# XiYe20/VPTR

Hardware: AMD Instinct MI355X
Metric: predicted frames/sec (train step) NAR KTH 10->10 @64x64 (higher is better)
Workload: dtype bf16x3 (split-bf16 MFMA, fp32 accumulate/storage); 1 GPU; K64: KTH 64x64x1 10->10, VPTREnc/Dec(528, Tanh, reflect) + VPTRFormerNAR(4 enc + 8 dec, d=528, 8 heads, ws 4, dropout 0.10), single_iter of train_NAR.py, random-init weights; per_gpu_batch=16, global_batch=16, frames_per_clip=10, parallelism=dp1, launch=hipGraph, dec_weight_grads=True, frozen_encoder_convs=winograd F(4x4,3x3), 36 strided-batch P16 products per convolution

## Files before the change

vptr_amd/_lib.py:

```python
import ctypes
import os

import torch

_HERE = os.path.dirname(os.path.abspath(__file__))
LIB_PATH = os.environ.get("VPTR_HIP_LIB") or os.path.join(_HERE, "libvptr_hip.so")

c_void_p, c_int, c_float, c_int64, c_uint32 = ctypes.c_void_p, ctypes.c_int, ctypes.c_float, ctypes.c_int64, ctypes.c_uint32


class GemmDesc(ctypes.Structure):
    _fields_ = [
        ("A", c_void_p), ("B", c_void_p), ("D", c_void_p), ("Dpre", c_void_p),
        ("lda", c_int64), ("ldb", c_int64), ("ldd", c_int64),
        ("M", c_int), ("N", c_int), ("K", c_int),
        ("a_mode", c_int), ("b_mode", c_int),
        ("precision", c_int), ("split_k", c_int), ("atomic", c_int),
        ("colscale", c_void_p), ("bias", c_void_p),
        ("alpha", c_float), ("act", c_int),
        ("rowscale", c_void_p), ("rs_div", c_int), ("rs_mod", c_int),
        ("dropout_p", c_float), ("seed_dev", c_void_p), ("site", c_uint32),
        ("residual", c_void_p), ("ldr", c_int64),
        ("act_after", c_int),
        ("conv_IH", c_int), ("conv_IW", c_int), ("conv_Cin", c_int), ("conv_OH", c_int), ("conv_OW", c_int),
        ("conv_KH", c_int), ("conv_KW", c_int), ("conv_stride", c_int), ("conv_pad", c_int), ("conv_pad_mode", c_int),
        ("conv_transposed", c_int),
        ("a_rowsum", c_void_p),
        ("batch", c_int), ("ksegs", c_int),
        ("A_x1", c_void_p), ("A_x2", c_void_p), ("B_x1", c_void_p), ("B_x2", c_void_p), ("D_x1", c_void_p), ("D_x2", c_void_p),
        ("bias_x1", c_void_p), ("bias_x2", c_void_p), ("alpha_x1", c_float), ("alpha_x2", c_float),
        ("D_planes", c_void_p),
        ("d_p16", c_int),
        ("act_grad_src", c_void_p),
        ("frame_stats", c_void_p), ("frame_rows", c_int),
        ("d_transposed", c_int),
        ("d_row_w", c_int), ("d_row_off", c_int),
        ("batch_accum", c_int),
        ("batch_stride_a", c_int64), ("batch_stride_b", c_int64), ("batch_stride_d", c_int64),
    ]


class ReduceEntry(ctypes.Structure):
    _fields_ = [("part", c_void_p), ("dst0", c_void_p), ("dst1", c_void_p), ("nparts", c_int), ("C", c_int)]


class WPlaneEntry(ctypes.Structure):
    _fields_ = [("W", c_void_p), ("Wp", c_void_p), ("WT", c_void_p), ("ldw", c_int64), ("N", c_int), ("K", c_int)]


P, I, F, L, U = c_void_p, c_int, c_float, c_int64, c_uint32
SIGNATURES = {
    "vptr_gemm": [ctypes.POINTER(GemmDesc), P],
    "vptr_gemm_tile_cols": [I],
    "vptr_split_planes": [P, P, L, I, P],
    "vptr_wino_in": [P, P, I, I, I, I, L, I, P],
    "vptr_wino_out": [P, P, P, P, P, I, I, I, I, L, I, I, P],
    "vptr_wino_out_in": [P, P, P, P, P, P, I, I, I, I, L, I, I, I, P],
    "vptr_to_p16": [P, P, L, I, P],
    "vptr_weight_planes": [P, P, I, I, P],
    "vptr_gemm_grouped": [ctypes.POINTER(GemmDesc), P, P, I, I, P],
    "vptr_layernorm_fwd": [P, P, P, P, P, P, I, I, P, P, I, I, F, I, P],
    "vptr_layernorm_bwd": [P, P, P, P, P, P, P, P, P, I, I, P, P],
    "vptr_layernorm_bwd_deferred": [P, P, P, P, P, P, P, I, I, P, P, P],
    "vptr_layernorm_bwd_partials": [I, I],
    "vptr_partial_reduce": [P, I, I, I, P],
    "vptr_rowmod_sum": [P, P, I, I, I, I, P],
    "vptr_colsum": [P, P, I, I, P],
    "vptr_window_copy": [P, P, I, I, I, I, I, I, I, I, P],
    "vptr_add_rowtab": [P, P, P, I, I, I, I, P],
    "vptr_winattn_fwd": [P, P, P, P, P, P, I, I, I, I, I, I, F, P, U, I, P],
    "vptr_winattn_bwd": [P, P, P, P, P, P, P, P, P, P, I, I, I, I, I, I, F, P, U, F, I, P],
    "vptr_winattn_bwd_ws": [P, P, P, P, P, P, P, P, P, P, I, I, I, I, I, I, F, P, U, F, I, P, I, P],
    "vptr_winattn_bwd_workspace": [I],
    "vptr_tattn_fwd": [P, P, P, P, I, I, I, I, I, I, I, F, P, U, I, P],
    "vptr_tattn_bwd": [P, P, P, P, P, P, P, I, I, I, I, I, I, I, F, P, U, F, I, P],
    "vptr_attn_route": [I, I, I, I, I, I, I, L, I, I, P, I],
    "vptr_tattn_step": [P, P, P, P, I, I, I, I, I, I, P],
    "vptr_tsattn_fwd": [P, P, P, P, I, I, I, I, I, I, I, I, F, P, U, I, P],
    "vptr_tsattn_bwd": [P, P, P, P, P, P, P, I, I, I, I, I, I, I, I, F, P, U, I, P],
    "vptr_colstats": [P, P, P, P, F, P, I, I, P],
    "vptr_colstats_running": [P, P, P, P, F, P, I, I, P, P, F, P, P],
    "vptr_groupstats": [P, P, P, P, F, I, I, P],
    "vptr_norm_act_fwd": [P, P, P, P, P, P, I, I, I, I, I, F, P, U, P, I, I, P, I, P, F, P],
    "vptr_norm_act_bwd": [P, P, P, P, P, P, P, P, P, P, I, I, I, I, I, I, F, P, U, P, I, I, I, P],
    "vptr_norm_act_bwd_deferred": [P, P, P, P, P, P, P, P, I, I, I, I, I, F, P, U, P, I, I, I, P, P],
    "vptr_norm_act_bwd_partials": [I, I, I, I],
    "vptr_dwconv3x3_fwd": [P, P, P, P, I, I, I, I, P, P],
    "vptr_dwconv3x3_bwd": [P, P, P, P, P, P, I, I, I, I, P],
    "vptr_dwconv3x3_norm_fwd": [P, P, P, P, F, I, P, P, P, P, P, P, I, I, I, I, P, P],
    "vptr_dwconv3x3_bwd_xh": [P, P, P, P, P, P, I, I, I, I, P],
    "vptr_nchw_to_tokens": [P, P, I, I, I, P],
    "vptr_tokens_to_nchw": [P, P, I, I, I, I, P],
    "vptr_nchw_to_tokens_masked": [P, P, P, I, I, I, P],
    "vptr_act_bwd": [P, P, P, I, I, I, F, P, I, I, F, P, U, I, P],
    "vptr_dropout": [P, P, L, F, P, U, P],
    "vptr_rowscale": [P, P, P, I, I, I, I, P],
    "vptr_conv7_in_fwd": [P, P, P, P, P, I, I, I, I, I, P],
    "vptr_conv7_in_fwd_planes": [P, P, P, P, P, I, I, I, I, I, P],
    "vptr_conv7_out_fwd": [P, P, P, P, I, I, I, I, I, I, P],
    "vptr_conv7_out_bwd_data": [P, P, P, P, I, I, I, I, I, I, P],
    "vptr_conv7_out_bwd_weight": [P, P, P, P, P, I, I, I, I, I, I, P],
    "vptr_conv7_out_bwd_weight_ws": [P, P, P, P, P, I, I, I, I, I, I, P, I, P],
    "vptr_conv7_out_bwd_weight_workspace": [I, I],
    "vptr_bnrelu_bwd": [P, P, P, P, L, I, P],
    "vptr_bnrelu_bwd_params": [P, P, P, P, P, P, L, I, P],
    "vptr_bnrelu_bwd_fused": [P, P, P, P, P, P, P, P, L, I, P],
    "vptr_im2col_nhwc": [P, P, I, I, I, I, I, I, I, I, I, I, I, P],
    "vptr_im2col_nhwc_p16": [P, P, I, I, I, I, I, I, I, I, I, I, I, P],
    "vptr_reflect_fold": [P, P, I, I, I, I, I, P],
    "vptr_conv7_in_bwd_weight": [P, P, P, I, I, I, I, I, P],
    "vptr_mse_gdl_fwd": [P, P, P, P, P, I, I, I, P],
    "vptr_mse_gdl_bwd": [P, P, P, P, P, I, I, I, P],
    "vptr_nce_fwd": [P, P, P, P, I, I, I, F, P],
    "vptr_nce_bwd": [P, P, P, P, P, P, I, I, I, F, P],
    "vptr_frame_metrics": [P, P, P, P, P, P, I, I, I, I, I, F, P],
    "vptr_frame_metrics_accumulate": [P, P, I, I, P],
    "vptr_clip_ingest": [P, P, P, P, P, P, P, P, P, I, I, I, I, I, I, I, I, I, I, I, I, I, I, P],
    "vptr_clip_panels": [P, P, P, P, P, P, P, P, I, I, I, I, I, I, I, I, I, P],
    "vptr_droppath_scales": [P, P, I, I, P, U, P],
    "vptr_sumsq": [P, L, P, P],
    "vptr_sumsq_ws": [P, L, P, P, I, P],
    "vptr_set_deterministic": [I],
    "vptr_get_deterministic": [],
    "vptr_wgrad_sync_stats": [P, P],
    "vptr_wgrad_kernel_counts": [P, I],
    "vptr_adamw": [P, P, P, P, L, F, F, F, F, F, P, P, F, F, P],
}
EXPORTS = sorted(list(SIGNATURES) + ["vptr_abi_version", "vptr_last_error"])
EXT_SIGNATURES = {
    "vptr_meters_add": [P, I, P, F, P],
}
OPTIM_SIGNATURES = {
    "vptr_optim_prepare": [P, P, P, P, P],
    "vptr_adamw_ctl": [P, P, P, P, L, P, P],
}
CONVFFN_SIGNATURES = {
    "vptr_norm_act_bwd_sums": [P, P, P, P, P, P, P, P, P, I, I, I, I, F, P, U, P, P],
    "vptr_dwconv3x3_norm_bwd": [P, P, P, P, P, P, P, I, F, P, U, P, P, P, P, P, I, I, I, I, I, P],
}


def _load():
    if not os.path.exists(LIB_PATH):
        raise ImportError(
            "vptr_amd: %s is missing. Build it with `python -m vptr_amd.build` (needs hipcc, gfx950). "
            "There is no CPU / PyTorch fallback for the VPTR hot path." % LIB_PATH)
    lib = ctypes.CDLL(LIB_PATH)
    for name, argt in list(SIGNATURES.items()) + list(EXT_SIGNATURES.items()) + list(OPTIM_SIGNATURES.items()) + list(CONVFFN_SIGNATURES.items()):
        fn = getattr(lib, name)
        fn.argtypes = argt
        fn.restype = c_int
    lib.vptr_abi_version.restype = c_int
    lib.vptr_last_error.restype = ctypes.c_char_p
    if lib.vptr_abi_version() != 10:
        raise ImportError("vptr_amd: ABI version mismatch in %s" % LIB_PATH)
    return lib


lib = _load()


def check(rc, what):
    if rc != 0:
        raise RuntimeError("%s failed (%d): %s" % (what, rc, lib.vptr_last_error().decode()))


def ptr(t):
    if t is None:
        return None
    return c_void_p(t.data_ptr())


def stream():
    return c_void_p(torch._C._cuda_getCurrentRawStream(torch.cuda.current_device()))


def require_cuda(*tensors):
    for t in tensors:
        if t is not None and not t.is_cuda:
            raise RuntimeError("vptr_amd ops run on the MI355X only (got a %s tensor); there is no CPU fallback" % t.device)
```

vptr_amd/build.py:

```python
import hashlib
import os
import subprocess
import sys
from concurrent.futures import ThreadPoolExecutor

HERE = os.path.dirname(os.path.abspath(__file__))
CSRC = os.path.join(HERE, "csrc")
OBJ = os.path.join(CSRC, "_build")
LIB = os.path.join(HERE, "libvptr_hip.so")
SOURCES = ["api.hip", "gemm.hip", "gemm_p16.hip", "layernorm.hip", "norm_act.hip", "dwconv.hip", "attn.hip", "attn_mfma.hip", "attn16.hip", "elementwise.hip", "conv7.hip", "losses.hip", "metrics.hip", "meters.hip", "optim.hip", "ingest.hip", "panels.hip", "winograd.hip"]
FLAGS = ["--offload-arch=gfx950", "-O3", "-std=c++17", "-fPIC", "-munsafe-fp-atomics", "-ffp-contract=fast", "-fno-slp-vectorize",
         "-Wno-unused-result"]


def _hipcc():
    for c in (os.environ.get("HIPCC"), "/opt/rocm/bin/hipcc", "hipcc"):
        if c and (os.path.isabs(c) and os.path.exists(c) or not os.path.isabs(c)):
            return c
    raise RuntimeError("hipcc not found")


def _digest(paths):
    h = hashlib.sha256()
    for p in paths:
        with open(p, "rb") as f:
            h.update(f.read())
    h.update(" ".join(FLAGS).encode())
    return h.hexdigest()


def _compile(src, force):
    obj = os.path.join(OBJ, src.replace(".hip", ".o"))
    stamp = obj + ".sha"
    deps = [os.path.join(CSRC, src), os.path.join(CSRC, "common.h"), os.path.join(CSRC, "gemm_shared.h"), os.path.join(CSRC, "attn_mfma.h"),
            os.path.join(CSRC, "attn_route.h"), os.path.join(HERE, "..", "include", "vptr_hip.h"), os.path.join(HERE, "..", "include", "vptr_hip_ext.h"),
            os.path.join(HERE, "..", "include", "vptr_hip_optim.h"), os.path.join(HERE, "..", "include", "vptr_hip_convffn.h")]
    dig = _digest(deps)
    if not force and os.path.exists(obj) and os.path.exists(stamp) and open(stamp).read() == dig:
        return obj, False
    cmd = [_hipcc()] + FLAGS + ["-c", os.path.join(CSRC, src), "-o", obj]
    r = subprocess.run(cmd, capture_output=True, text=True)
    if r.returncode != 0:
        raise RuntimeError("hipcc failed for %s:\n%s\n%s" % (src, r.stdout[-4000:], r.stderr[-8000:]))
    with open(stamp, "w") as f:
        f.write(dig)
    return obj, True


def build(force=False, verbose=True):
    os.makedirs(OBJ, exist_ok=True)
    with ThreadPoolExecutor(max_workers=min(8, len(SOURCES))) as ex:
        res = list(ex.map(lambda s: _compile(s, force), SOURCES))
    objs = [o for o, _ in res]
    if any(c for _, c in res) or not os.path.exists(LIB):
        cmd = [_hipcc(), "--offload-arch=gfx950", "-shared", "-fPIC", "-o", LIB] + objs
        r = subprocess.run(cmd, capture_output=True, text=True)
        if r.returncode != 0:
            raise RuntimeError("link failed:\n%s\n%s" % (r.stdout[-4000:], r.stderr[-8000:]))
        if verbose:
            print("built", LIB)
    elif verbose:
        print("up to date:", LIB)
    return LIB


if __name__ == "__main__":
    build(force="--force" in sys.argv)
```

vptr_amd/csrc/dwconv.hip:

```cpp
#include "common.h"
#include "../../include/vptr_hip_convffn.h"
#include <type_traits>

struct DwRow { float4 l, m, r; };
__device__ __forceinline__ float4 scale4(const float4 v, const float s) { return make_float4(v.x * s, v.y * s, v.z * s, v.w * s); }
__device__ __forceinline__ DwRow dw_load_row(const float4* __restrict__ x, int64_t frame_row0, int row, int H, int xw, int W, int F4,
                                             int c4) {
  const float rok = (row >= 0 && row < H) ? 1.f : 0.f;
  const int64_t base = (frame_row0 + min(max(row, 0), H - 1)) * W;
  DwRow o;
  o.l = scale4(x[(base + max(xw - 1, 0)) * F4 + c4], xw > 0 ? rok : 0.f);
  o.m = scale4(x[(base + xw) * F4 + c4], rok);
  o.r = scale4(x[(base + min(xw + 1, W - 1)) * F4 + c4], xw + 1 < W ? rok : 0.f);
  return o;
}
__device__ __forceinline__ void fma4(float4& a, const float4 w, const float4 v) {
  a.x += w.x * v.x; a.y += w.y * v.y; a.z += w.z * v.z; a.w += w.w * v.w;
}
__global__ __launch_bounds__(256) void dwconv_fwd_kernel(const float* __restrict__ x_, const float* __restrict__ w9,
                                                         const float* __restrict__ b, float* __restrict__ y_, int frames, int H,
                                                         int W, int F4, int flip) {
  const int64_t idx = (int64_t)blockIdx.x * 256 + threadIdx.x;
  if (idx >= (int64_t)frames * W * F4) return;
  const int c4 = (int)(idx % F4);
  const int xw = (int)((idx / F4) % W);
  const int64_t f = idx / ((int64_t)F4 * W);
  const float4* __restrict__ x = reinterpret_cast<const float4*>(x_);
  float4* __restrict__ y = reinterpret_cast<float4*>(y_);
  float4 w[9];
#pragma unroll
  for (int t = 0; t < 9; ++t) w[t] = reinterpret_cast<const float4*>(w9)[(int64_t)(flip ? 8 - t : t) * F4 + c4];
  const float4 bias = b ? reinterpret_cast<const float4*>(b)[c4] : make_float4(0.f, 0.f, 0.f, 0.f);
  DwRow r0 = dw_load_row(x, f * H, -1, H, xw, W, F4, c4), r1 = dw_load_row(x, f * H, 0, H, xw, W, F4, c4);
  for (int yh = 0; yh < H; ++yh) {
    const DwRow r2 = dw_load_row(x, f * H, yh + 1, H, xw, W, F4, c4);
    float4 a = bias;
    fma4(a, w[0], r0.l); fma4(a, w[1], r0.m); fma4(a, w[2], r0.r);
    fma4(a, w[3], r1.l); fma4(a, w[4], r1.m); fma4(a, w[5], r1.r);
    fma4(a, w[6], r2.l); fma4(a, w[7], r2.m); fma4(a, w[8], r2.r);
    y[((f * H + yh) * W + xw) * F4 + c4] = a;
    r0 = r1;
    r1 = r2;
  }
}

struct DwRow2 { float4 c0, c1, c2, c3; };
typedef __attribute__((ext_vector_type(4))) _Float16 half4_t;
__device__ __forceinline__ float4 dw_ld4(const float4* __restrict__ x, const int64_t i) { return x[i]; }
__device__ __forceinline__ float4 dw_ld4(const half4_t* __restrict__ x, const int64_t i) {
  const half4_t h = x[i];
  return make_float4((float)h.x, (float)h.y, (float)h.z, (float)h.w);
}
template <typename XT>
__device__ __forceinline__ DwRow2 dw_load_row2(const XT* __restrict__ x, int64_t frame_row0, int row, int H, int xw0, int W, int F4,
                                               int c4) {
  const float rok = (row >= 0 && row < H) ? 1.f : 0.f;
  const int64_t base = (frame_row0 + min(max(row, 0), H - 1)) * W;
  DwRow2 o;
  o.c0 = scale4(dw_ld4(x, (base + max(xw0 - 1, 0)) * F4 + c4), xw0 > 0 ? rok : 0.f);
  o.c1 = scale4(dw_ld4(x, (base + xw0) * F4 + c4), rok);
  o.c2 = scale4(dw_ld4(x, (base + xw0 + 1) * F4 + c4), rok);
  o.c3 = scale4(dw_ld4(x, (base + min(xw0 + 2, W - 1)) * F4 + c4), xw0 + 2 < W ? rok : 0.f);
  return o;
}
__global__ __launch_bounds__(256) void dwconv_fwd2_kernel(const float* __restrict__ x_, const float* __restrict__ w9,
                                                          const float* __restrict__ b, float* __restrict__ y_, int frames, int H,
                                                          int W, int F4, int flip, float* __restrict__ stats) {
  const int64_t idx = (int64_t)blockIdx.x * 256 + threadIdx.x;
  const int W2 = W >> 1;
  if (idx >= (int64_t)frames * W2 * F4) return;
  const int c4 = (int)(idx % F4);
  const int xw0 = (int)((idx / F4) % W2) * 2;
  const int64_t f = idx / ((int64_t)F4 * W2);
  const float4* __restrict__ x = reinterpret_cast<const float4*>(x_);
  float4* __restrict__ y = reinterpret_cast<float4*>(y_);
  float4 w[9];
#pragma unroll
  for (int t = 0; t < 9; ++t) w[t] = reinterpret_cast<const float4*>(w9)[(int64_t)(flip ? 8 - t : t) * F4 + c4];
  const float4 bias = b ? reinterpret_cast<const float4*>(b)[c4] : make_float4(0.f, 0.f, 0.f, 0.f);
  DwRow2 r0 = dw_load_row2(x, f * H, -1, H, xw0, W, F4, c4), r1 = dw_load_row2(x, f * H, 0, H, xw0, W, F4, c4);
  float ssum = 0.f, ssq = 0.f;
  for (int yh = 0; yh < H; ++yh) {
    const DwRow2 r2 = dw_load_row2(x, f * H, yh + 1, H, xw0, W, F4, c4);
    float4 a = bias, a2 = bias;
    fma4(a, w[0], r0.c0); fma4(a, w[1], r0.c1); fma4(a, w[2], r0.c2);
    fma4(a, w[3], r1.c0); fma4(a, w[4], r1.c1); fma4(a, w[5], r1.c2);
    fma4(a, w[6], r2.c0); fma4(a, w[7], r2.c1); fma4(a, w[8], r2.c2);
    fma4(a2, w[0], r0.c1); fma4(a2, w[1], r0.c2); fma4(a2, w[2], r0.c3);
    fma4(a2, w[3], r1.c1); fma4(a2, w[4], r1.c2); fma4(a2, w[5], r1.c3);
    fma4(a2, w[6], r2.c1); fma4(a2, w[7], r2.c2); fma4(a2, w[8], r2.c3);
    y[((f * H + yh) * W + xw0) * F4 + c4] = a;
    y[((f * H + yh) * W + xw0 + 1) * F4 + c4] = a2;
    if (stats) {
      ssum += ((a.x + a.y) + (a.z + a.w)) + ((a2.x + a2.y) + (a2.z + a2.w));
      ssq += ((a.x * a.x + a.y * a.y) + (a.z * a.z + a.w * a.w)) + ((a2.x * a2.x + a2.y * a2.y) + (a2.z * a2.z + a2.w * a2.w));
    }
    r0 = r1;
    r1 = r2;
  }
  if (stats) {
    const float S = wave_sum(ssum), Q = wave_sum(ssq);
    if ((threadIdx.x & 63) == 0) {
      unsafeAtomicAdd(stats + VPTR_FRAME_STATS_STRIDE * f, S);
      unsafeAtomicAdd(stats + VPTR_FRAME_STATS_STRIDE * f + 1, Q);
    }
  }
}
__device__ __forceinline__ float dpp_from_prev(float v) {
  return __int_as_float(__builtin_amdgcn_update_dpp(0, __float_as_int(v), 0x111, 0xf, 0xf, true));
}
__device__ __forceinline__ float dpp_from_next(float v) {
  return __int_as_float(__builtin_amdgcn_update_dpp(0, __float_as_int(v), 0x101, 0xf, 0xf, true));
}
__device__ __forceinline__ DwRow2 dw_load_row3(const float4* __restrict__ x, int64_t frame_row0, int row, int H, int xw0, int W, int F4,
                                               int c4, float lok, float rok_) {
  const float rok = (row >= 0 && row < H) ? 1.f : 0.f;
  const int64_t base = (frame_row0 + min(max(row, 0), H - 1)) * W;
  DwRow2 o;
  o.c1 = scale4(x[(base + xw0) * F4 + c4], rok);
  o.c2 = scale4(x[(base + xw0 + 1) * F4 + c4], rok);
  o.c0 = make_float4(dpp_from_prev(o.c2.x) * lok, dpp_from_prev(o.c2.y) * lok, dpp_from_prev(o.c2.z) * lok, dpp_from_prev(o.c2.w) * lok);
  o.c3 = make_float4(dpp_from_next(o.c1.x) * rok_, dpp_from_next(o.c1.y) * rok_, dpp_from_next(o.c1.z) * rok_, dpp_from_next(o.c1.w) * rok_);
  return o;
}
__global__ __launch_bounds__(256) void dwconv_fwd3_kernel(const float* __restrict__ x_, const float* __restrict__ w9,
                                                          const float* __restrict__ b, float* __restrict__ y_, int frames, int H,
                                                          int W, int F4, int flip, float* __restrict__ stats) {
  const int64_t idx = (int64_t)blockIdx.x * 256 + threadIdx.x;
  const int W2 = W >> 1;
  if (idx >= (int64_t)frames * W2 * F4) return;
  const int xp = (int)(idx % W2), xw0 = xp * 2;
  const int c4 = (int)((idx / W2) % F4);
  const int64_t f = idx / ((int64_t)F4 * W2);
  const float lok = xp > 0 ? 1.f : 0.f, rok_ = xp + 1 < W2 ? 1.f : 0.f;
  const float4* __restrict__ x = reinterpret_cast<const float4*>(x_);
  float4* __restrict__ y = reinterpret_cast<float4*>(y_);
  float4 w[9];
#pragma unroll
  for (int t = 0; t < 9; ++t) w[t] = reinterpret_cast<const float4*>(w9)[(int64_t)(flip ? 8 - t : t) * F4 + c4];
  const float4 bias = b ? reinterpret_cast<const float4*>(b)[c4] : make_float4(0.f, 0.f, 0.f, 0.f);
  DwRow2 r0 = dw_load_row3(x, f * H, -1, H, xw0, W, F4, c4, lok, rok_), r1 = dw_load_row3(x, f * H, 0, H, xw0, W, F4, c4, lok, rok_);
  float ssum = 0.f, ssq = 0.f;
  for (int yh = 0; yh < H; ++yh) {
    const DwRow2 r2 = dw_load_row3(x, f * H, yh + 1, H, xw0, W, F4, c4, lok, rok_);
    float4 a = bias, a2 = bias;
    fma4(a, w[0], r0.c0); fma4(a, w[1], r0.c1); fma4(a, w[2], r0.c2);
    fma4(a, w[3], r1.c0); fma4(a, w[4], r1.c1); fma4(a, w[5], r1.c2);
    fma4(a, w[6], r2.c0); fma4(a, w[7], r2.c1); fma4(a, w[8], r2.c2);
    fma4(a2, w[0], r0.c1); fma4(a2, w[1], r0.c2); fma4(a2, w[2], r0.c3);
    fma4(a2, w[3], r1.c1); fma4(a2, w[4], r1.c2); fma4(a2, w[5], r1.c3);
    fma4(a2, w[6], r2.c1); fma4(a2, w[7], r2.c2); fma4(a2, w[8], r2.c3);
    y[((f * H + yh) * W + xw0) * F4 + c4] = a;
    y[((f * H + yh) * W + xw0 + 1) * F4 + c4] = a2;
    if (stats) {
      ssum += ((a.x + a.y) + (a.z + a.w)) + ((a2.x + a2.y) + (a2.z + a2.w));
      ssq += ((a.x * a.x + a.y * a.y) + (a.z * a.z + a.w * a.w)) + ((a2.x * a2.x + a2.y * a2.y) + (a2.z * a2.z + a2.w * a2.w));
    }
    r0 = r1;
    r1 = r2;
  }
  if (stats) {
    const float S = wave_sum(ssum), Q = wave_sum(ssq);
    if ((threadIdx.x & 63) == 0) {
      unsafeAtomicAdd(stats + VPTR_FRAME_STATS_STRIDE * f, S);
      unsafeAtomicAdd(stats + VPTR_FRAME_STATS_STRIDE * f + 1, Q);
    }
  }
}
__device__ __forceinline__ float4 dwn_act4(const float4 v, const float m, const float r, const float4 w, const float4 b, const int act, const float ok) {
  float4 o;
  o.x = vptr_act((v.x - m) * r * w.x + b.x, act) * ok;
  o.y = vptr_act((v.y - m) * r * w.y + b.y, act) * ok;
  o.z = vptr_act((v.z - m) * r * w.z + b.z, act) * ok;
  o.w = vptr_act((v.w - m) * r * w.w + b.w, act) * ok;
  return o;
}
__device__ __forceinline__ void dwn_store_half4(_Float16* __restrict__ ah, const int64_t e, const float4 v) {
  const half4_t h = {(_Float16)v.x, (_Float16)v.y, (_Float16)v.z, (_Float16)v.w};
  *reinterpret_cast<half4_t*>(ah + e) = h;
}
__global__ __launch_bounds__(256) void dwconv_norm_fwd3_kernel(const float* __restrict__ x_, const float* __restrict__ raw_stats,
                                                               const float* __restrict__ aw_, const float* __restrict__ ab_, float eps, int act,
                                                               const float* __restrict__ w9, const float* __restrict__ b, float* __restrict__ y_,
                                                               _Float16* __restrict__ ah, float* __restrict__ mean_out, float* __restrict__ rstd_out,
                                                               int frames, int H, int W, int F4, float* __restrict__ stats) {
  const int64_t idx = (int64_t)blockIdx.x * 256 + threadIdx.x;
  const int W2 = W >> 1;
  if (idx >= (int64_t)frames * W2 * F4) return;
  const int xp = (int)(idx % W2), xw0 = xp * 2;
  const int c4 = (int)((idx / W2) % F4);
  const int64_t f = idx / ((int64_t)F4 * W2);
  const float lok = xp > 0 ? 1.f : 0.f, rok_ = xp + 1 < W2 ? 1.f : 0.f;
  const float4* __restrict__ x = reinterpret_cast<const float4*>(x_);
  const float4* __restrict__ aw = reinterpret_cast<const float4*>(aw_);
  const float4* __restrict__ ab = reinterpret_cast<const float4*>(ab_);
  float4* __restrict__ y = reinterpret_cast<float4*>(y_);
  const int P = H * W * F4;
  const float inv_n = 1.f / ((float)P * 4.f);
  float m = raw_stats[VPTR_FRAME_STATS_STRIDE * f] * inv_n;
  const float e2 = raw_stats[VPTR_FRAME_STATS_STRIDE * f + 1] * inv_n;
  float var = fmaxf(e2 - m * m, 0.f);
  if (var < 1e-2f * e2) {
    const float4* xf = x + f * P;
    float sq = 0.f, s1 = 0.f;
    for (int j = threadIdx.x & 63; j < P; j += 64) {
      const float4 t = xf[j];
      const float a = t.x - m, b2 = t.y - m, c = t.z - m, d = t.w - m;
      s1 += (a + b2) + (c + d);
      sq += (a * a + b2 * b2) + (c * c + d * d);
    }
    const float dm = wave_sum(s1) * inv_n;
    var = fmaxf(wave_sum(sq) * inv_n - dm * dm, 0.f);
    m += dm;
  }
  const float r = rsqrtf(var + eps);
  if (xp == 0 && c4 == 0) { mean_out[f] = m; rstd_out[f] = r; }
  float4 w[9];
#pragma unroll
  for (int t = 0; t < 9; ++t) w[t] = reinterpret_cast<const float4*>(w9)[(int64_t)t * F4 + c4];
  const float4 bias = b ? reinterpret_cast<const float4*>(b)[c4] : make_float4(0.f, 0.f, 0.f, 0.f);
  struct Raw { float4 x1, x2, w1, w2, b1, b2; };
  auto fetch = [&](const int row) -> Raw {
    const int rc = min(max(row, 0), H - 1);
    const int64_t base = ((f * H + rc) * W + xw0) * F4 + c4;
    const int hw = (rc * W + xw0) * F4 + c4;
    Raw q;
    q.x1 = x[base]; q.x2 = x[base + F4];
    q.w1 = aw[hw]; q.w2 = aw[hw + F4]; q.b1 = ab[hw]; q.b2 = ab[hw + F4];
    return q;
  };
  auto activate = [&](const Raw& q, const int row) -> DwRow2 {
    const bool in = row >= 0 && row < H;
    const float rok = in ? 1.f : 0.f;
    DwRow2 o;
    o.c1 = dwn_act4(q.x1, m, r, q.w1, q.b1, act, rok);
    o.c2 = dwn_act4(q.x2, m, r, q.w2, q.b2, act, rok);
    if (ah && in) {
      const int64_t base = ((f * H + row) * W + xw0) * F4 + c4;
      dwn_store_half4(ah, base * 4, o.c1);
      dwn_store_half4(ah, (base + F4) * 4, o.c2);
    }
    o.c0 = make_float4(dpp_from_prev(o.c2.x) * lok, dpp_from_prev(o.c2.y) * lok, dpp_from_prev(o.c2.z) * lok, dpp_from_prev(o.c2.w) * lok);
    o.c3 = make_float4(dpp_from_next(o.c1.x) * rok_, dpp_from_next(o.c1.y) * rok_, dpp_from_next(o.c1.z) * rok_, dpp_from_next(o.c1.w) * rok_);
    return o;
  };
  Raw q1 = fetch(0), q2 = fetch(1);
  DwRow2 r0, r1 = activate(q1, 0);
  r0.c0 = r0.c1 = r0.c2 = r0.c3 = make_float4(0.f, 0.f, 0.f, 0.f);
  float ssum = 0.f, ssq = 0.f;
  for (int yh = 0; yh < H; ++yh) {
    const Raw q3 = fetch(yh + 2);
    const DwRow2 r2 = activate(q2, yh + 1);
    float4 a = bias, a2 = bias;
    fma4(a, w[0], r0.c0); fma4(a, w[1], r0.c1); fma4(a, w[2], r0.c2);
    fma4(a, w[3], r1.c0); fma4(a, w[4], r1.c1); fma4(a, w[5], r1.c2);
    fma4(a, w[6], r2.c0); fma4(a, w[7], r2.c1); fma4(a, w[8], r2.c2);
    fma4(a2, w[0], r0.c1); fma4(a2, w[1], r0.c2); fma4(a2, w[2], r0.c3);
    fma4(a2, w[3], r1.c1); fma4(a2, w[4], r1.c2); fma4(a2, w[5], r1.c3);
    fma4(a2, w[6], r2.c1); fma4(a2, w[7], r2.c2); fma4(a2, w[8], r2.c3);
    y[((f * H + yh) * W + xw0) * F4 + c4] = a;
    y[((f * H + yh) * W + xw0 + 1) * F4 + c4] = a2;
    if (stats) {
      ssum += ((a.x + a.y) + (a.z + a.w)) + ((a2.x + a2.y) + (a2.z + a2.w));
      ssq += ((a.x * a.x + a.y * a.y) + (a.z * a.z + a.w * a.w)) + ((a2.x * a2.x + a2.y * a2.y) + (a2.z * a2.z + a2.w * a2.w));
    }
    r0 = r1;
    r1 = r2;
    q2 = q3;
  }
  if (stats) {
    const float S = wave_sum(ssum), Q = wave_sum(ssq);
    if ((threadIdx.x & 63) == 0) {
      unsafeAtomicAdd(stats + VPTR_FRAME_STATS_STRIDE * f, S);
      unsafeAtomicAdd(stats + VPTR_FRAME_STATS_STRIDE * f + 1, Q);
    }
  }
}
__global__ __launch_bounds__(256) void dwconv_norm_lds_kernel(const float* __restrict__ x_, const float* __restrict__ raw_stats,
                                                              const float* __restrict__ aw_, const float* __restrict__ ab_, float eps, int act,
                                                              const float* __restrict__ w9, const float* __restrict__ b, float* __restrict__ y_,
                                                              _Float16* __restrict__ ah, float* __restrict__ mean_out, float* __restrict__ rstd_out,
                                                              int H, int W, int F4, float* __restrict__ stats) {
  extern __shared__ float4 dwn_tile[];
  const int tid = threadIdx.x, c4l = tid & 15, p0 = tid >> 4;
  const int c4 = blockIdx.x * 16 + c4l;
  const int64_t f = blockIdx.y;
  const int HW = H * W;
  const float4* __restrict__ x = reinterpret_cast<const float4*>(x_);
  const float4* __restrict__ aw = reinterpret_cast<const float4*>(aw_);
  const float4* __restrict__ ab = reinterpret_cast<const float4*>(ab_);
  float4* __restrict__ y = reinterpret_cast<float4*>(y_);
  const int P = HW * F4;
  const float inv_n = 1.f / ((float)P * 4.f);
  float m = raw_stats[VPTR_FRAME_STATS_STRIDE * f] * inv_n;
  const float e2 = raw_stats[VPTR_FRAME_STATS_STRIDE * f + 1] * inv_n;
  float var = fmaxf(e2 - m * m, 0.f);
  if (var < 1e-2f * e2) {
    const float4* xf = x + f * P;
    float sq = 0.f, s1 = 0.f;
    for (int j = tid & 63; j < P; j += 64) {
      const float4 t = xf[j];
      const float a = t.x - m, b2 = t.y - m, c = t.z - m, d = t.w - m;
      s1 += (a + b2) + (c + d);
      sq += (a * a + b2 * b2) + (c * c + d * d);
    }
    const float dm = wave_sum(s1) * inv_n;
    var = fmaxf(wave_sum(sq) * inv_n - dm * dm, 0.f);
    m += dm;
  }
  const float r = rsqrtf(var + eps);
  if (tid == 0 && blockIdx.x == 0) { mean_out[f] = m; rstd_out[f] = r; }
  float4 w[9];
#pragma unroll
  for (int t = 0; t < 9; ++t) w[t] = reinterpret_cast<const float4*>(w9)[(int64_t)t * F4 + c4];
  const float4 bias = b ? reinterpret_cast<const float4*>(b)[c4] : make_float4(0.f, 0.f, 0.f, 0.f);
  for (int pb = 0; pb < HW; pb += 64) {
    float4 xv[4], wv[4], bv[4];
#pragma unroll
    for (int k = 0; k < 4; ++k) {
      const int p = min(pb + p0 + 16 * k, HW - 1);
      xv[k] = x[(f * HW + p) * F4 + c4];
      wv[k] = aw[(int64_t)p * F4 + c4];
      bv[k] = ab[(int64_t)p * F4 + c4];
    }
#pragma unroll
    for (int k = 0; k < 4; ++k) {
      const int p = pb + p0 + 16 * k;
      if (p < HW) {
        const float4 a = dwn_act4(xv[k], m, r, wv[k], bv[k], act, 1.f);
        dwn_tile[p * 16 + c4l] = a;
        if (ah) dwn_store_half4(ah, ((f * HW + p) * F4 + c4) * 4, a);
      }
    }
  }
  __syncthreads();
  float ssum = 0.f, ssq = 0.f;
  for (int p = p0; p < HW; p += 16) {
    const int py = p / W, px = p - py * W;
    float4 a = bias;
#pragma unroll
    for (int ky = 0; ky < 3; ++ky) {
      const int yy = py + ky - 1;
      const bool yok = yy >= 0 && yy < H;
#pragma unroll
      for (int kx = 0; kx < 3; ++kx) {
        const int xx = px + kx - 1;
        const bool ok = yok && xx >= 0 && xx < W;
        const float4 v = dwn_tile[(ok ? yy * W + xx : p) * 16 + c4l];
        fma4(a, w[ky * 3 + kx], scale4(v, ok ? 1.f : 0.f));
      }
    }
    y[(f * HW + p) * F4 + c4] = a;
    ssum += (a.x + a.y) + (a.z + a.w);
    ssq += (a.x * a.x + a.y * a.y) + (a.z * a.z + a.w * a.w);
  }
  if (stats) {
    __shared__ float dwn_red[8];
    const float S = wave_sum(ssum), Q = wave_sum(ssq);
    if ((tid & 63) == 0) { dwn_red[tid >> 6] = S; dwn_red[4 + (tid >> 6)] = Q; }
    __syncthreads();
    if (tid == 0) {
      unsafeAtomicAdd(stats + VPTR_FRAME_STATS_STRIDE * f, (dwn_red[0] + dwn_red[1]) + (dwn_red[2] + dwn_red[3]));
      unsafeAtomicAdd(stats + VPTR_FRAME_STATS_STRIDE * f + 1, (dwn_red[4] + dwn_red[5]) + (dwn_red[6] + dwn_red[7]));
    }
  }
}
extern "C" int vptr_dwconv3x3_norm_fwd(const float* x, const float* raw_stats, const float* aff_w, const float* aff_b, float eps, int act,
                                       const float* w9, const float* b, float* y, void* a_half, float* mean_out, float* rstd_out,
                                       int frames, int H, int W, int F, float* frame_stats, vptr_stream_t stream) {
  VPTR_CHECK(x && raw_stats && aff_w && aff_b && w9 && y && mean_out && rstd_out && frames > 0 && H > 0 && W > 0 && F > 0 && F % 4 == 0,
             "dwconv3x3_norm_fwd: bad arguments");
  const int W2 = W / 2;
  VPTR_CHECK(W % 2 == 0 && W2 >= 1 && 16 % W2 == 0 && (W2 * (F / 4)) % 64 == 0,
             "dwconv3x3_norm_fwd: needs W even, W / 2 dividing 16 and (W/2)*(F/4) %% 64 == 0 (got W %d, F %d)", W, F);
  VPTR_CHECK(((reinterpret_cast<uintptr_t>(x) | reinterpret_cast<uintptr_t>(y) | reinterpret_cast<uintptr_t>(aff_w) | reinterpret_cast<uintptr_t>(aff_b) |
               reinterpret_cast<uintptr_t>(w9) | reinterpret_cast<uintptr_t>(b)) & 15) == 0 && (reinterpret_cast<uintptr_t>(a_half) & 7) == 0,
             "dwconv3x3_norm_fwd: operands must be 16-byte aligned");
  if (F % 64 == 0 && H * W <= 256 && frames <= 65535) {
    dwconv_norm_lds_kernel<<<dim3(F / 64, frames), 256, (size_t)H * W * 256, (hipStream_t)stream>>>(
        x, raw_stats, aff_w, aff_b, eps, act, w9, b, y, reinterpret_cast<_Float16*>(a_half), mean_out, rstd_out, H, W, F / 4, frame_stats);
    VPTR_LAUNCH_CHECK();
    return 0;
  }
  const int64_t total = (int64_t)frames * W2 * (F / 4);
  dwconv_norm_fwd3_kernel<<<(unsigned)((total + 255) / 256), 256, 0, (hipStream_t)stream>>>(
      x, raw_stats, aff_w, aff_b, eps, act, w9, b, y, reinterpret_cast<_Float16*>(a_half), mean_out, rstd_out, frames, H, W, F / 4, frame_stats);
  VPTR_LAUNCH_CHECK();
  return 0;
}

__device__ __forceinline__ float4 norm_act_dx4(const float4 dv, const float4 xv, const float4 ww, const float4 bb, const float mu, const float rs,
                                               const float t1, const float t2, const float inv_n, const int act, const bool drop, const float p,
                                               const uint64_t seed, const uint32_t site, const uint64_t e0) {
  const float xs[4] = {xv.x, xv.y, xv.z, xv.w}, ds4[4] = {dv.x, dv.y, dv.z, dv.w};
  const float wv[4] = {ww.x, ww.y, ww.z, ww.w}, bv[4] = {bb.x, bb.y, bb.z, bb.w};
  float o[4];
#pragma unroll
  for (int u = 0; u < 4; ++u) {
    const float xh = (xs[u] - mu) * rs;
    const float dsc = drop ? vptr_drop_scale(seed, site, e0 + u, p) : 1.f;
    const float g = norm_act_g(ds4[u], xh, wv[u], bv[u], act, dsc);
    o[u] = rs * (g * wv[u] - t1 * inv_n - xh * t2 * inv_n);
  }
  return make_float4(o[0], o[1], o[2], o[3]);
}
template <int ACT, bool DROP>
__global__ __launch_bounds__(256) void dwconv_norm_bwd_lds_kernel(const float4* __restrict__ dy, const float4* __restrict__ y2,
                                                                  const float* __restrict__ mean2, const float* __restrict__ rstd2,
                                                                  const float4* __restrict__ w2, const float4* __restrict__ b2,
                                                                  const float* __restrict__ fsum, int act_rt, float p,
                                                                  const uint64_t* __restrict__ seed_dev, uint32_t site,
                                                                  const half4_t* __restrict__ ah, const float4* __restrict__ w9,
                                                                  float4* __restrict__ da, float* __restrict__ dw9, float* __restrict__ db,
                                                                  int frames, int H, int W, int F4, int fpb) {
  extern __shared__ float4 dwb_tile[];
  const int act = ACT >= 0 ? ACT : act_rt;
  const int tid = threadIdx.x, c4l = tid & 15, p0 = tid >> 4;
  const int c4 = blockIdx.x * 16 + c4l;
  const int HW = H * W, Wp = W + 2, P = HW * F4;
  const int f0 = blockIdx.y * fpb, f1 = min(frames, f0 + fpb);
  uint64_t seed = 0;
  if (DROP) seed = *seed_dev;
  const float inv_n = 1.f / (float)((int64_t)HW * F4 * 4);
  for (int i = tid; i < (H + 2) * Wp * 16; i += 256) dwb_tile[i] = make_float4(0.f, 0.f, 0.f, 0.f);
  int pos[4], ctr[4], dst[4];
  bool ok[4];
  float4 wv[4], bv[4];
#pragma unroll
  for (int k = 0; k < 4; ++k) {
    const int pk = p0 + 16 * k;
    ok[k] = pk < HW;
    const int pc = min(pk, HW - 1), py = pc / W, px = pc - py * W;
    pos[k] = pc * F4 + c4;
    ctr[k] = ((py + 1) * Wp + px + 1) * 16 + c4l;
    dst[k] = ok[k] ? ctr[k] : (H + 2) * Wp * 16 + c4l;
    wv[k] = w2[pos[k]];
    bv[k] = b2[pos[k]];
  }
  float4 wf[9], acc[9], ab = make_float4(0.f, 0.f, 0.f, 0.f);
#pragma unroll
  for (int t = 0; t < 9; ++t) {
    wf[t] = w9[(int64_t)(8 - t) * F4 + c4];
    acc[t] = make_float4(0.f, 0.f, 0.f, 0.f);
  }
  float4 dv[4], yv[4];
  half4_t av[4];
#pragma unroll
  for (int k = 0; k < 4; ++k) {
    const int64_t i = (int64_t)f0 * P + pos[k];
    dv[k] = dy[i];
    yv[k] = y2[i];
    av[k] = ah[i];
  }
  __syncthreads();
  for (int f = f0; f < f1; ++f) {
    const float mu = mean2[f], rs = rstd2[f], t1 = fsum[f], t2 = fsum[frames + f];
    const int64_t base = (int64_t)f * P;
    const int64_t nbase = (int64_t)min(f + 1, f1 - 1) * P;
    float4 nd[4], ny[4];
    half4_t na[4];
#pragma unroll
    for (int k = 0; k < 4; ++k) {
      nd[k] = dy[nbase + pos[k]];
      ny[k] = y2[nbase + pos[k]];
      na[k] = ah[nbase + pos[k]];
    }
    __builtin_amdgcn_sched_barrier(0);
    half4_t a[4];
#pragma unroll
    for (int k = 0; k < 4; ++k) {
      dwb_tile[dst[k]] = norm_act_dx4(dv[k], yv[k], wv[k], bv[k], mu, rs, t1, t2, inv_n, act, DROP, p, seed, site, (uint64_t)(base + pos[k]) * 4);
      a[k] = av[k];
    }
    __syncthreads();
#pragma unroll
    for (int k = 0; k < 4; ++k) {
      if (!ok[k]) continue;
      const float4 af = make_float4((float)a[k].x, (float)a[k].y, (float)a[k].z, (float)a[k].w);
      float4 o = make_float4(0.f, 0.f, 0.f, 0.f);
#pragma unroll
      for (int ky = 0; ky < 3; ++ky)
#pragma unroll
        for (int kx = 0; kx < 3; ++kx) {
          const float4 v = dwb_tile[ctr[k] + ((ky - 1) * Wp + (kx - 1)) * 16];
          fma4(o, wf[ky * 3 + kx], v);
          fma4(acc[ky * 3 + kx], af, v);
          if (ky == 1 && kx == 1) { ab.x += v.x; ab.y += v.y; ab.z += v.z; ab.w += v.w; }
        }
      da[base + pos[k]] = o;
    }
#pragma unroll
    for (int k = 0; k < 4; ++k) { dv[k] = nd[k]; yv[k] = ny[k]; av[k] = na[k]; }
    __syncthreads();
  }
  auto lanes4 = [](float4& v) {
    v.x += __shfl_xor(v.x, 16, 64); v.y += __shfl_xor(v.y, 16, 64); v.z += __shfl_xor(v.z, 16, 64); v.w += __shfl_xor(v.w, 16, 64);
    v.x += __shfl_xor(v.x, 32, 64); v.y += __shfl_xor(v.y, 32, 64); v.z += __shfl_xor(v.z, 32, 64); v.w += __shfl_xor(v.w, 32, 64);
  };
#pragma unroll
  for (int t = 0; t < 9; ++t) lanes4(acc[t]);
  lanes4(ab);
  const int wave = tid >> 6;
  if ((tid & 63) < 16) {
#pragma unroll
    for (int t = 0; t < 9; ++t) dwb_tile[(wave * 10 + t) * 16 + c4l] = acc[t];
    dwb_tile[(wave * 10 + 9) * 16 + c4l] = ab;
  }
  __syncthreads();
  const float* red = reinterpret_cast<const float*>(dwb_tile);
  const int F = F4 * 4;
  for (int o = tid; o < 640; o += 256) {
    const int r = o >> 6, ch = o & 63;
    const float sum = (red[r * 64 + ch] + red[(10 + r) * 64 + ch]) + (red[(20 + r) * 64 + ch] + red[(30 + r) * 64 + ch]);
    if (r < 9) unsafeAtomicAdd(dw9 + (int64_t)(8 - r) * F + blockIdx.x * 64 + ch, sum);
    else unsafeAtomicAdd(db + blockIdx.x * 64 + ch, sum);
  }
}
extern "C" int vptr_dwconv3x3_norm_bwd(const float* dy, const float* y2, const float* mean2, const float* rstd2, const float* w2, const float* b2,
                                       const float* fsum, int act, float dropout_p, const uint64_t* seed_dev, uint32_t site, const void* a_half,
                                       const float* w9, float* da, float* dw9, float* db, int frames, int H, int W, int F, int frames_per_group,
                                       vptr_stream_t stream) {
  VPTR_CHECK(dy && y2 && mean2 && rstd2 && w2 && b2 && fsum && a_half && w9 && da && dw9 && db && frames > 0 && H > 0 && W > 0 && F > 0 &&
                 frames_per_group >= 0,
             "dwconv3x3_norm_bwd: bad arguments");
  VPTR_CHECK(!g_vptr_deterministic, "dwconv3x3_norm_bwd: workgroups meet in atomics; the deterministic mode takes vptr_norm_act_bwd + vptr_dwconv3x3_bwd_xh");
  const int W2 = W / 2;
  VPTR_CHECK(F % 64 == 0 && W % 2 == 0 && W2 >= 1 && 16 % W2 == 0 && (W2 * (F / 4)) % 64 == 0,
             "dwconv3x3_norm_bwd: needs F %% 64 == 0, W even, W / 2 dividing 16 and (W/2)*(F/4) %% 64 == 0 (got W %d, F %d)", W, F);
  VPTR_CHECK((int64_t)H * W <= 64, "dwconv3x3_norm_bwd: maps of at most 64 pixels (got %d x %d)", H, W);
  VPTR_CHECK(dropout_p >= 0.f && dropout_p < 1.f && (dropout_p == 0.f || seed_dev), "dwconv3x3_norm_bwd: dropout needs 0 <= p < 1 and seed_dev");
// ... 144 lines not shown
```

Measured before the change: 3644 frames/s.

## Process several frames per block in dwconv-norm forward with prefetch and double-buffered LDS

Adds a grouped variant of the fused norm+activation+depthwise 3x3 forward kernel for small spatial sizes (H*W<=64). Each block loops over a group of frames, chosen from the CU count, and keeps the affine weights, conv weights and bias in registers across them. It prefetches the next frame's input, double-buffers the LDS tile and defers the per-frame stats atomics, so one barrier per frame suffices. Templating on activation and half output removes runtime branches. The cost is fewer blocks, which lowers parallelism when the frame count is small, and more LDS per block.

```diff
diff --git a/include/vptr_hip_convffn_ext.h b/include/vptr_hip_convffn_ext.h
--- /dev/null
+++ b/include/vptr_hip_convffn_ext.h
@@ -0,0 +1,18 @@
+#ifndef VPTR_HIP_CONVFFN_EXT_H
+#define VPTR_HIP_CONVFFN_EXT_H
+
+#include "vptr_hip.h"
+
+#ifdef __cplusplus
+extern "C" {
+#endif
+
+int vptr_dwconv3x3_norm_fwd_g(const float* x, const float* raw_stats, const float* aff_w, const float* aff_b, float eps, int act,
+                              const float* w9, const float* b, float* y, void* a_half, float* mean_out, float* rstd_out,
+                              int frames, int H, int W, int F, float* frame_stats, int frames_per_group, vptr_stream_t stream);
+
+#ifdef __cplusplus
+}
+#endif
+
+#endif
diff --git a/vptr_amd/_lib.py b/vptr_amd/_lib.py
--- a/vptr_amd/_lib.py
+++ b/vptr_amd/_lib.py
@@ -138,6 +138,9 @@
     "vptr_norm_act_bwd_sums": [P, P, P, P, P, P, P, P, P, I, I, I, I, F, P, U, P, P],
     "vptr_dwconv3x3_norm_bwd": [P, P, P, P, P, P, P, I, F, P, U, P, P, P, P, P, I, I, I, I, I, P],
 }
+CONVFFN_EXT_SIGNATURES = {
+    "vptr_dwconv3x3_norm_fwd_g": SIGNATURES["vptr_dwconv3x3_norm_fwd"][:-1] + [I, P],
+}
 
 
 def _load():
@@ -146,7 +149,8 @@
             "vptr_amd: %s is missing. Build it with `python -m vptr_amd.build` (needs hipcc, gfx950). "
             "There is no CPU / PyTorch fallback for the VPTR hot path." % LIB_PATH)
     lib = ctypes.CDLL(LIB_PATH)
-    for name, argt in list(SIGNATURES.items()) + list(EXT_SIGNATURES.items()) + list(OPTIM_SIGNATURES.items()) + list(CONVFFN_SIGNATURES.items()):
+    for name, argt in (list(SIGNATURES.items()) + list(EXT_SIGNATURES.items()) + list(OPTIM_SIGNATURES.items()) + list(CONVFFN_SIGNATURES.items()) +
+                       list(CONVFFN_EXT_SIGNATURES.items())):
         fn = getattr(lib, name)
         fn.argtypes = argt
         fn.restype = c_int
diff --git a/vptr_amd/build.py b/vptr_amd/build.py
--- a/vptr_amd/build.py
+++ b/vptr_amd/build.py
@@ -34,7 +34,8 @@
     stamp = obj + ".sha"
     deps = [os.path.join(CSRC, src), os.path.join(CSRC, "common.h"), os.path.join(CSRC, "gemm_shared.h"), os.path.join(CSRC, "attn_mfma.h"),
             os.path.join(CSRC, "attn_route.h"), os.path.join(HERE, "..", "include", "vptr_hip.h"), os.path.join(HERE, "..", "include", "vptr_hip_ext.h"),
-            os.path.join(HERE, "..", "include", "vptr_hip_optim.h"), os.path.join(HERE, "..", "include", "vptr_hip_convffn.h")]
+            os.path.join(HERE, "..", "include", "vptr_hip_optim.h"), os.path.join(HERE, "..", "include", "vptr_hip_convffn.h"),
+            os.path.join(HERE, "..", "include", "vptr_hip_convffn_ext.h")]
     dig = _digest(deps)
     if not force and os.path.exists(obj) and os.path.exists(stamp) and open(stamp).read() == dig:
         return obj, False
diff --git a/vptr_amd/csrc/dwconv.hip b/vptr_amd/csrc/dwconv.hip
--- a/vptr_amd/csrc/dwconv.hip
+++ b/vptr_amd/csrc/dwconv.hip
@@ -1,5 +1,6 @@
 #include "common.h"
 #include "../../include/vptr_hip_convffn.h"
+#include "../../include/vptr_hip_convffn_ext.h"
 #include <type_traits>
 
 struct DwRow { float4 l, m, r; };
@@ -276,6 +277,27 @@
     }
   }
 }
+__device__ __forceinline__ void dwn_slab_frame_stats(const float4* __restrict__ x, const float* __restrict__ raw_stats, const int64_t f, const int P,
+                                                     const float inv_n, const float eps, const int tid, float& m_out, float& r_out) {
+  float m = raw_stats[VPTR_FRAME_STATS_STRIDE * f] * inv_n;
+  const float e2 = raw_stats[VPTR_FRAME_STATS_STRIDE * f + 1] * inv_n;
+  float var = fmaxf(e2 - m * m, 0.f);
+  if (var < 1e-2f * e2) {
+    const float4* xf = x + f * P;
+    float sq = 0.f, s1 = 0.f;
+    for (int j = tid & 63; j < P; j += 64) {
+      const float4 t = xf[j];
+      const float a = t.x - m, b2 = t.y - m, c = t.z - m, d = t.w - m;
+      s1 += (a + b2) + (c + d);
+      sq += (a * a + b2 * b2) + (c * c + d * d);
+    }
+    const float dm = wave_sum(s1) * inv_n;
+    var = fmaxf(wave_sum(sq) * inv_n - dm * dm, 0.f);
+    m += dm;
+  }
+  m_out = m;
+  r_out = rsqrtf(var + eps);
+}
 __global__ __launch_bounds__(256) void dwconv_norm_lds_kernel(const float* __restrict__ x_, const float* __restrict__ raw_stats,
                                                               const float* __restrict__ aw_, const float* __restrict__ ab_, float eps, int act,
                                                               const float* __restrict__ w9, const float* __restrict__ b, float* __restrict__ y_,
@@ -292,23 +314,8 @@
   float4* __restrict__ y = reinterpret_cast<float4*>(y_);
   const int P = HW * F4;
   const float inv_n = 1.f / ((float)P * 4.f);
-  float m = raw_stats[VPTR_FRAME_STATS_STRIDE * f] * inv_n;
-  const float e2 = raw_stats[VPTR_FRAME_STATS_STRIDE * f + 1] * inv_n;
-  float var = fmaxf(e2 - m * m, 0.f);
-  if (var < 1e-2f * e2) {
-    const float4* xf = x + f * P;
-    float sq = 0.f, s1 = 0.f;
-    for (int j = tid & 63; j < P; j += 64) {
-      const float4 t = xf[j];
-      const float a = t.x - m, b2 = t.y - m, c = t.z - m, d = t.w - m;
-      s1 += (a + b2) + (c + d);
-      sq += (a * a + b2 * b2) + (c * c + d * d);
-    }
-    const float dm = wave_sum(s1) * inv_n;
-    var = fmaxf(wave_sum(sq) * inv_n - dm * dm, 0.f);
-    m += dm;
-  }
-  const float r = rsqrtf(var + eps);
+  float m, r;
+  dwn_slab_frame_stats(x, raw_stats, f, P, inv_n, eps, tid, m, r);
   if (tid == 0 && blockIdx.x == 0) { mean_out[f] = m; rstd_out[f] = r; }
   float4 w[9];
 #pragma unroll
@@ -365,10 +372,120 @@
     }
   }
 }
+static int dwn_fwd_group(int slabs, int frames) {
+  static int cus = -1;
+  if (cus < 0) {
+    int dev = 0, v = 0;
+    cus = (hipGetDevice(&dev) == hipSuccess && hipDeviceGetAttribute(&v, hipDeviceAttributeMultiprocessorCount, dev) == hipSuccess) ? v : 0;
+  }
+  if (cus <= 0) return 8;
+  int best = 8;
+  for (int g = 7; g >= 4; --g)
+    if (cdiv((int64_t)slabs * cdiv(frames, g), cus) * g < cdiv((int64_t)slabs * cdiv(frames, best), cus) * best) best = g;
+  return best;
+}
+template <int ACT, bool HALF>
+__global__ __launch_bounds__(256) void dwconv_norm_lds_grp_kernel(const float* __restrict__ x_, const float* __restrict__ raw_stats,
+                                                                  const float* __restrict__ aw_, const float* __restrict__ ab_, float eps, int act_rt,
+                                                                  const float* __restrict__ w9, const float* __restrict__ b, float* __restrict__ y_,
+                                                                  _Float16* __restrict__ ah, float* __restrict__ mean_out, float* __restrict__ rstd_out,
+                                                                  int frames, int H, int W, int F4, float* __restrict__ stats, int fpg) {
+  extern __shared__ float4 dwn_tile[];
+  __shared__ float dwn_red2[2][8];
+  const int act = ACT >= 0 ? ACT : act_rt;
+  const int tid = threadIdx.x, c4l = tid & 15, p0 = tid >> 4;
+  const int c4 = blockIdx.x * 16 + c4l;
+  const int HW = H * W;
+  const int f0 = blockIdx.y * fpg, f1 = min(frames, f0 + fpg);
+  const float4* __restrict__ x = reinterpret_cast<const float4*>(x_);
+  const float4* __restrict__ aw = reinterpret_cast<const float4*>(aw_);
+  const float4* __restrict__ ab = reinterpret_cast<const float4*>(ab_);
+  float4* __restrict__ y = reinterpret_cast<float4*>(y_);
+  const int P = HW * F4;
+  const float inv_n = 1.f / ((float)P * 4.f);
+  float4 w[9];
+#pragma unroll
+  for (int t = 0; t < 9; ++t) w[t] = reinterpret_cast<const float4*>(w9)[(int64_t)t * F4 + c4];
+  const float4 bias = b ? reinterpret_cast<const float4*>(b)[c4] : make_float4(0.f, 0.f, 0.f, 0.f);
+  int pos[4];
+  float4 wv[4], bv[4], xv[4];
+#pragma unroll
+  for (int k = 0; k < 4; ++k) {
+    const int p = min(p0 + 16 * k, HW - 1);
+    pos[k] = p * F4 + c4;
+    wv[k] = aw[pos[k]];
+    bv[k] = ab[pos[k]];
+    xv[k] = x[(int64_t)f0 * P + pos[k]];
+  }
+  auto add_stats = [&](const int f) {
+    const float* red = dwn_red2[f & 1];
+    unsafeAtomicAdd(stats + VPTR_FRAME_STATS_STRIDE * (int64_t)f, (red[0] + red[1]) + (red[2] + red[3]));
+    unsafeAtomicAdd(stats + VPTR_FRAME_STATS_STRIDE * (int64_t)f + 1, (red[4] + red[5]) + (red[6] + red[7]));
+  };
+  for (int fi = f0; fi < f1; ++fi) {
+    const int64_t f = fi;
+    float4* __restrict__ tile = dwn_tile + (fi & 1) * HW * 16;
+    const int64_t nbase = (int64_t)min(fi + 1, f1 - 1) * P;
+    float4 nx[4];
+#pragma unroll
+    for (int k = 0; k < 4; ++k) nx[k] = x[nbase + pos[k]];
+    __builtin_amdgcn_sched_barrier(0);
+    float m, r;
+    dwn_slab_frame_stats(x, raw_stats, f, P, inv_n, eps, tid, m, r);
+    if (tid == 0 && blockIdx.x == 0) { mean_out[f] = m; rstd_out[f] = r; }
+#pragma unroll
+    for (int k = 0; k < 4; ++k) {
+      const int p = p0 + 16 * k;
+      if (p < HW) {
+        const float4 a = dwn_act4(xv[k], m, r, wv[k], bv[k], act, 1.f);
+        tile[p * 16 + c4l] = a;
+        if (HALF) dwn_store_half4(ah, (f * P + pos[k]) * 4, a);
+      }
+    }
+    __syncthreads();
+    if (stats && tid == 0 && fi > f0) add_stats(fi - 1);
+    float ssum = 0.f, ssq = 0.f;
+    for (int p = p0; p < HW; p += 16) {
+      const int py = p / W, px = p - py * W;
+      float4 a = bias;
+#pragma unroll
+      for (int ky = 0; ky < 3; ++ky) {
+        const int yy = py + ky - 1;
+        const bool yok = yy >= 0 && yy < H;
+#pragma unroll
+        for (int kx = 0; kx < 3; ++kx) {
+          const int xx = px + kx - 1;
+          const bool ok = yok && xx >= 0 && xx < W;
+          const float4 v = tile[(ok ? yy * W + xx : p) * 16 + c4l];
+          fma4(a, w[ky * 3 + kx], scale4(v, ok ? 1.f : 0.f));
+        }
+      }
+      y[(f * HW + p) * F4 + c4] = a;
+      ssum += (a.x + a.y) + (a.z + a.w);
+      ssq += (a.x * a.x + a.y * a.y) + (a.z * a.z + a.w * a.w);
+    }
+    if (stats) {
+      const float S = wave_sum(ssum), Q = wave_sum(ssq);
+      if ((tid & 63) == 0) { dwn_red2[fi & 1][tid >> 6] = S; dwn_red2[fi & 1][4 + (tid >> 6)] = Q; }
+    }
+#pragma unroll
+    for (int k = 0; k < 4; ++k) xv[k] = nx[k];
+  }
+  if (stats) {
+    __syncthreads();
+    if (tid == 0) add_stats(f1 - 1);
+  }
+}
 extern "C" int vptr_dwconv3x3_norm_fwd(const float* x, const float* raw_stats, const float* aff_w, const float* aff_b, float eps, int act,
                                        const float* w9, const float* b, float* y, void* a_half, float* mean_out, float* rstd_out,
                                        int frames, int H, int W, int F, float* frame_stats, vptr_stream_t stream) {
-  VPTR_CHECK(x && raw_stats && aff_w && aff_b && w9 && y && mean_out && rstd_out && frames > 0 && H > 0 && W > 0 && F > 0 && F % 4 == 0,
+  return vptr_dwconv3x3_norm_fwd_g(x, raw_stats, aff_w, aff_b, eps, act, w9, b, y, a_half, mean_out, rstd_out, frames, H, W, F, frame_stats, 0, stream);
+}
+extern "C" int vptr_dwconv3x3_norm_fwd_g(const float* x, const float* raw_stats, const float* aff_w, const float* aff_b, float eps, int act,
+                                         const float* w9, const float* b, float* y, void* a_half, float* mean_out, float* rstd_out,
+                                         int frames, int H, int W, int F, float* frame_stats, int frames_per_group, vptr_stream_t stream) {
+  VPTR_CHECK(x && raw_stats && aff_w && aff_b && w9 && y && mean_out && rstd_out && frames > 0 && H > 0 && W > 0 && F > 0 && F % 4 == 0 &&
+                 frames_per_group >= 0,
              "dwconv3x3_norm_fwd: bad arguments");
   const int W2 = W / 2;
   VPTR_CHECK(W % 2 == 0 && W2 >= 1 && 16 % W2 == 0 && (W2 * (F / 4)) % 64 == 0,
@@ -376,6 +493,16 @@
   VPTR_CHECK(((reinterpret_cast<uintptr_t>(x) | reinterpret_cast<uintptr_t>(y) | reinterpret_cast<uintptr_t>(aff_w) | reinterpret_cast<uintptr_t>(aff_b) |
                reinterpret_cast<uintptr_t>(w9) | reinterpret_cast<uintptr_t>(b)) & 15) == 0 && (reinterpret_cast<uintptr_t>(a_half) & 7) == 0,
              "dwconv3x3_norm_fwd: operands must be 16-byte aligned");
+  if (F % 64 == 0 && H * W <= 64 && frames <= 65535) {
+    const int fpg = frames_per_group ? frames_per_group : (frames >= 64 ? dwn_fwd_group(F / 64, frames) : 1);
+    const bool gelu = act == VPTR_ACT_GELU;
+    auto kern = gelu ? (a_half ? dwconv_norm_lds_grp_kernel<VPTR_ACT_GELU, true> : dwconv_norm_lds_grp_kernel<VPTR_ACT_GELU, false>)
+                     : (a_half ? dwconv_norm_lds_grp_kernel<-1, true> : dwconv_norm_lds_grp_kernel<-1, false>);
+    kern<<<dim3(F / 64, cdiv(frames, fpg)), 256, (size_t)H * W * 512, (hipStream_t)stream>>>(
+        x, raw_stats, aff_w, aff_b, eps, act, w9, b, y, reinterpret_cast<_Float16*>(a_half), mean_out, rstd_out, frames, H, W, F / 4, frame_stats, fpg);
+    VPTR_LAUNCH_CHECK();
+    return 0;
+  }
   if (F % 64 == 0 && H * W <= 256 && frames <= 65535) {
     dwconv_norm_lds_kernel<<<dim3(F / 64, frames), 256, (size_t)H * W * 256, (hipStream_t)stream>>>(
         x, raw_stats, aff_w, aff_b, eps, act, w9, b, y, reinterpret_cast<_Float16*>(a_half), mean_out, rstd_out, H, W, F / 4, frame_stats);
```

Result: no change. 3643 frames/s (-0.0%).
